# quan-dao/practical-collab-perception

Hardware: AMD Instinct MI355X
Metric: frames/sec (60k-pt cloud, 6 agents) (higher is better)
Workload: dtype f32

## Files before the change

include/pcp_hip.h:

```cpp
#ifndef PCP_HIP_H
#define PCP_HIP_H

#include <stddef.h>
#include <stdint.h>

#ifdef __cplusplus
extern "C" {
#endif

#define PCP_ABI_VERSION 1

enum {
  PCP_OK = 0,
  PCP_ERR_ARG = 1,
  PCP_ERR_WORKSPACE = 2,
  PCP_ERR_LAUNCH = 3,
  PCP_ERR_UNSUPPORTED = 4
};

int pcp_abi_version(void);
const char *pcp_status_string(int status);

enum {
  PCP_OPT_PFN_CROWD = 0,
  PCP_OPT_PFN_CROWD_BLOCKS = 1,
  PCP_OPT_PFN_WPS = 2,
  PCP_OPT_WINO4C_NW = 3,
  PCP_OPT_MP_TH16_MIN = 4,
  PCP_OPT_MP_DIAG = 5,
  PCP_OPT_VOX_AGGREGATE = 6,
  PCP_OPT_CONV_S2_FORM = 7,
  PCP_OPT_COUNT = 8
};
int pcp_set_option(int32_t option, int64_t value);
int64_t pcp_get_option(int32_t option);

typedef struct {
  float min_x, min_y, min_z;
  float voxel_x, voxel_y, voxel_z;
  int32_t nx, ny;
  int32_t batch_size;
} pcp_grid_t;

#define PCP_VOX_COUNTERS 4

size_t pcp_voxelize_workspace_bytes(const pcp_grid_t *grid, int64_t max_points);

int pcp_voxelize(const float *points, int64_t n, int32_t row_stride, const pcp_grid_t *grid,
                 void *workspace, size_t workspace_bytes,
                 int32_t *voxel_coords, int64_t *unq_inv, int32_t *unq_cnt, int32_t *counters, void *stream);
int pcp_voxelize_cells_ready(const float *points, int64_t n, int32_t row_stride, const pcp_grid_t *grid,
                             void *workspace, size_t workspace_bytes,
                             int32_t *voxel_coords, int32_t *unq_cnt, int32_t *counters, void *stream);

int pcp_voxelize_sort_pillar_rows(const pcp_grid_t *grid, void *workspace, int64_t n, void *stream);
int pcp_voxelize_row_order(const pcp_grid_t *grid, const void *workspace, int64_t n, int32_t *order, int32_t *cursor_scratch,
                           void *stream);

int pcp_pfn_scatter(const float *points, int64_t n, int32_t row_stride, int32_t num_raw, const pcp_grid_t *grid,
                    const void *workspace, const float *w0, const float *b0, const float *w1, const float *b1,
                    float *pillar_features, float *canvas, void *stream);

#define PCP_ROWS_CELLS_READY 1
#define PCP_ROWS_BUCKET_ORDER 2
size_t pcp_pillarise_rows_workspace_bytes(const pcp_grid_t *grid, int64_t max_points, int32_t num_raw);
int pcp_pillarise_rows(const float *points, int64_t n, int32_t row_stride, int32_t num_raw, const pcp_grid_t *grid,
                       void *workspace, size_t workspace_bytes, int32_t *voxel_coords, int64_t *unq_inv, int32_t *unq_cnt,
                       int32_t *counters, int32_t flags, void *stream);
int pcp_pfn_rows(const pcp_grid_t *grid, const void *workspace, int64_t n, int32_t num_raw, const float *w0, const float *b0,
                 const float *w1, const float *b1, float *pillar_features, float *canvas, void *stream);
int pcp_pillar_index_export(const pcp_grid_t *grid, const void *workspace, int64_t n, int32_t num_raw, int32_t *voxel_coords,
                            int32_t *row_rank, int32_t *slot_rank, int32_t *slot_canvas_row, int32_t *counters, void *stream);

#define PCP_PFN_ABSOLUTE_XYZ 1u
#define PCP_PFN_WITH_DISTANCE 2u
int pcp_pfn_features(const float *points, int64_t n, int32_t row_stride, int32_t num_raw, uint32_t flags, const pcp_grid_t *grid,
                     const void *vox_workspace, int32_t fw, float *fbuf, int32_t *slot_pillar, void *stream);
int pcp_pfn_cat_pillar_max(const float *y, int32_t ld_y, const float *pillar_max, int32_t ld_max, const int32_t *slot_pillar, int64_t rows,
                           int32_t c, float *out, int32_t ld_out, void *stream);

int pcp_canvas_clear(const pcp_grid_t *grid, const void *workspace, int64_t n, float *canvas, void *stream);
int pcp_fill_zero(void *ptr, size_t bytes, void *stream);

typedef struct {
  int32_t batch, in_h, in_w;
  int32_t cin, cout;
  int32_t cout_pad;
  int32_t stride;
  int32_t ld_in, ld_out;
  int32_t relu;
} pcp_conv3x3_t;

int pcp_conv3x3(const pcp_conv3x3_t *desc, const float *in, const float *w_packed, const float *bias, float *out,
                void *stream);

int pcp_sparse_conv3x3_s2(const float *pillar_features, const pcp_grid_t *grid, const void *vox_workspace, int64_t n,
                          const float *w_packed, const float *bias, int32_t cout, int32_t relu, float *out, int32_t ld_out,
                          void *stream);

int pcp_conv3x3_winograd(const pcp_conv3x3_t *desc, const float *in, const float *u_packed, const float *bias, float *out,
                         void *stream);

int pcp_conv3x3_winograd_ws_supported(const pcp_conv3x3_t *desc);
int pcp_conv3x3_winograd_ws(const pcp_conv3x3_t *desc, const float *in, const float *u_packed, const float *bias, float *out,
                            void *stream);
int pcp_conv3x3_winograd_ws_plan(const pcp_conv3x3_t *desc, int32_t *variant, double *executed_flops);

int pcp_conv3x3_winograd4f(const pcp_conv3x3_t *desc, const float *in, const float *u_packed, const float *bias, float *out,
                           void *stream);
int pcp_conv3x3_winograd4f_plan(const pcp_conv3x3_t *desc, double *executed_flops);

int pcp_conv3x3_winograd4h(const pcp_conv3x3_t *desc, const float *in, const float *u_packed, const float *bias, float *out,
                           void *stream);
int pcp_conv3x3_winograd4h_plan(const pcp_conv3x3_t *desc, double *executed_flops);

// ... 199 lines not shown
```

practical-collab-perception_amd/csrc/abi.hip:

```cpp
#include "pcp_common.h"

extern "C" int pcp_abi_version(void) { return PCP_ABI_VERSION; }

extern "C" const char *pcp_status_string(int status) {
  switch (status) {
    case PCP_OK: return "ok";
    case PCP_ERR_ARG: return "bad argument";
    case PCP_ERR_WORKSPACE: return "workspace too small";
    case PCP_ERR_LAUNCH: return "kernel launch failed";
    case PCP_ERR_UNSUPPORTED: return "unsupported shape for this build";
    default: return "unknown status";
  }
}

#include <atomic>

namespace {
std::atomic<long long> g_option[PCP_OPT_COUNT] = {{-1}, {-1}, {-1}, {-1}, {-1}, {-1}, {-1}, {-1}};
static_assert(PCP_OPT_COUNT == 8, "one initialiser per option");
constexpr int MAX_DEVICES = 64;
std::atomic<int> g_cus[MAX_DEVICES];
}

extern "C" int pcp_set_option(int32_t option, int64_t value) {
  if (option < 0 || option >= PCP_OPT_COUNT) return PCP_ERR_ARG;
  g_option[option].store(value < 0 ? -1 : (long long)value, std::memory_order_relaxed);
  return PCP_OK;
}

extern "C" int64_t pcp_get_option(int32_t option) {
  if (option < 0 || option >= PCP_OPT_COUNT) return -1;
  return g_option[option].load(std::memory_order_relaxed);
}

long long pcp_option(int option, long long builtin) {
  const long long v = g_option[option].load(std::memory_order_relaxed);
  return v < 0 ? builtin : v;
}

int pcp_current_device_cus() {
  int dev = 0;
  if (hipGetDevice(&dev) != hipSuccess || dev < 0 || dev >= MAX_DEVICES) return 256;
  int v = g_cus[dev].load(std::memory_order_relaxed);
  if (v > 0) return v;
  if (hipDeviceGetAttribute(&v, hipDeviceAttributeMultiprocessorCount, dev) != hipSuccess || v <= 0) v = 256;
  g_cus[dev].store(v, std::memory_order_relaxed);
  return v;
}
```

practical-collab-perception_amd/csrc/conv.hip:

```cpp
#include "pcp_common.h"

namespace {

constexpr int CK = 16;
constexpr int LDK = 20;
constexpr int CONV_THREADS = 256;

__device__ __forceinline__ int xcd_remap(int bid, int nwg) {
  const int q = nwg >> 3, r = nwg & 7, x = bid & 7;
  return (x < r ? x * (q + 1) : r * (q + 1) + (x - r) * q) + (bid >> 3);
}

__device__ __forceinline__ f32x16 mfma32(float a, float b, f32x16 c) {
  return __builtin_amdgcn_mfma_f32_32x32x2f32(a, b, c, 0, 0, 0);
}

struct Conv3Params {
  const float *in;
  const float *w;
  const float *bias;
  float *out;
  int batch, in_h, in_w, out_h, out_w;
  int cin, cout, cout_pad;
  int ld_in, ld_out;
// ... 269 lines not shown
  f32x4 af[2][MI];
  patch_load(0);
#pragma unroll
  for (int t = 0; t < W2_RING; t++) wr[t] = w_load(0, t);
  patch_store(0);
  patch_load(1);
  __syncthreads();
  for (int slice = 0; slice < n_slices; slice++) {
    const float *As = lds + (slice & 1) * BUF;
    patch_store((slice + 1) & 1);
    patch_load(slice + 2);
#pragma unroll
    for (int i = 0; i < MI; i++) af[0][i] = *reinterpret_cast<const f32x4 *>(As + a_off[i][0]);
    fence();
#pragma unroll
    for (int t = 0; t < 18; t++) {
      if (t + 1 < 18) {
#pragma unroll
        for (int i = 0; i < MI; i++)
          af[(t + 1) & 1][i] = *reinterpret_cast<const f32x4 *>(As + (a_off[i][(t + 1) >> 1] ^ (((t + 1) & 1) * 8)));
      }
      if (t > 0) wr[(t - 1) % W2_RING] = w_load(slice + (t - 1 + W2_RING >= 18 ? 1 : 0), (t - 1 + W2_RING) % 18);
      fence();
      const f32x4 bf = wr[t % W2_RING];
      const f32x4 a0 = af[t & 1][0], a1 = af[t & 1][1];
      acc[0] = mfma32(bf.x, a0.x, acc[0]);
      acc[1] = mfma32(bf.x, a1.x, acc[1]);
      acc[0] = mfma32(bf.y, a0.y, acc[0]);
      acc[1] = mfma32(bf.y, a1.y, acc[1]);
      acc[0] = mfma32(bf.z, a0.z, acc[0]);
      acc[1] = mfma32(bf.z, a1.z, acc[1]);
      acc[0] = mfma32(bf.w, a0.w, acc[0]);
      acc[1] = mfma32(bf.w, a1.w, acc[1]);
      fence();
    }
    wr[17 % W2_RING] = w_load(slice + 1, (17 + W2_RING) % 18);
    __syncthreads();
  }

  const int nb = n0 + wn * 32;
#pragma unroll
  for (int i = 0; i < MI; i++) {
    const int m = wm * 64 + i * 32 + r;
    const int oy = oy0 + m / TW, ox = ox0 + m % TW;
    if (oy >= p.out_h || ox >= p.out_w) continue;
    float *orow = p.out + ((long long)(b * p.out_h + oy) * p.out_w + ox) * p.ld_out;
#pragma unroll
    for (int q = 0; q < 4; q++) {
      const int co = nb + 8 * q + 4 * h;
      if (co >= p.cout) continue;
      const f32x4 bias = *reinterpret_cast<const f32x4 *>(p.bias + co);
      f32x4 v = f32x4{acc[i][4 * q], acc[i][4 * q + 1], acc[i][4 * q + 2], acc[i][4 * q + 3]} + bias;
      if (p.relu) {
        v.x = fmaxf(v.x, 0.f); v.y = fmaxf(v.y, 0.f); v.z = fmaxf(v.z, 0.f); v.w = fmaxf(v.w, 0.f);
      }
      if (co + 3 < p.cout && p.vec_out) {
        *reinterpret_cast<f32x4 *>(orow + co) = v;
      } else {
        orow[co] = v.x;
        if (co + 1 < p.cout) orow[co + 1] = v.y;
        if (co + 2 < p.cout) orow[co + 2] = v.z;
        if (co + 3 < p.cout) orow[co + 3] = v.w;
      }
    }
  }
}

struct PwParams {
  const float *in;
  const float *in2;
  const float *residual;
  int ld_in2, k_split, ld_res;
  const float *w;
  const float *bias;
  float *out;
  long long rows;
  int in_h, in_w;
  int cin, cout, cout_pad, n_total;
  int k_total;
  int ld_in, ld_out;
  int relu;
  int n_tiles;
  int vec_out;
};

template <int MODE, int BM, int BN, int WAVES_M, int WAVES_N>
__global__ __launch_bounds__(CONV_THREADS, 2) void k_pointwise(PwParams p) {
  constexpr int WTM = BM / WAVES_M, WTN = BN / WAVES_N;
  constexpr int MI = WTM / 32, NI = WTN / 32;
  constexpr int A_F4 = BM * (CK / 4), B_F4 = BN * (CK / 4);
  constexpr int A_PER = (A_F4 + CONV_THREADS - 1) / CONV_THREADS;
  constexpr int B_PER = (B_F4 + CONV_THREADS - 1) / CONV_THREADS;
  __shared__ __attribute__((aligned(16))) float lds[(BM + BN) * LDK];
  float *As = lds;
  float *Bs = lds + BM * LDK;

  const int tid = threadIdx.x, lane = tid & 63, wave = tid >> 6;
  const int r = lane & 31, h = lane >> 5;
  const int wm = wave / WAVES_N, wn = wave % WAVES_N;
  const int lid = xcd_remap(blockIdx.x, gridDim.x);
  const int nt = lid % p.n_tiles;
  const long long m0 = (long long)(lid / p.n_tiles) * BM;
  const int n0 = nt * BN;

  const float *a_row[A_PER];
  const float *a_row2[A_PER];
  int a_dst[A_PER];
#pragma unroll
  for (int i = 0; i < A_PER; i++) {
    int idx = tid + i * CONV_THREADS;
    a_row[i] = nullptr;
    a_row2[i] = nullptr;
    a_dst[i] = -1;
    if (idx < A_F4) {
      int row = idx >> 2, q = idx & 3;
      long long m = m0 + row;
      a_dst[i] = row * LDK + q * 4;
      if (m < p.rows) {
        if (MODE == PCP_PW_PLAIN && p.in2) a_row2[i] = p.in2 + m * p.ld_in2 + q * 4;
        if (MODE == PCP_PW_SPACE2DEPTH) {
          int ow = p.in_w >> 1, oh = p.in_h >> 1;
          int ox = (int)(m % ow);
          long long t = m / ow;
          int oy = (int)(t % oh), bb = (int)(t / oh);
          a_row[i] = p.in + ((long long)(bb * p.in_h + 2 * oy) * p.in_w + 2 * ox) * p.ld_in + q * 4;
        } else {
          a_row[i] = p.in + m * p.ld_in + q * 4;
        }
      }
    }
  }
  int b_goff[B_PER], b_dst[B_PER];
#pragma unroll
  for (int i = 0; i < B_PER; i++) {
    int idx = tid + i * CONV_THREADS;
    b_dst[i] = -1;
    b_goff[i] = 0;
    if (idx < B_F4) {
      int n = idx >> 2, q = idx & 3;
      b_goff[i] = (n0 + n) * CK + q * 4;
      b_dst[i] = n * LDK + q * 4;
    }
  }
  const int slices_per_tap = p.cin / CK;
  f32x4 a_reg[A_PER], b_reg[B_PER];
  auto load_slice = [&](int slice) {
    int tap = 0, c0 = slice * CK;
    long long tap_off = 0;
    if (MODE == PCP_PW_SPACE2DEPTH) {
      tap = slice / slices_per_tap;
      c0 = (slice % slices_per_tap) * CK;
      tap_off = ((long long)(tap >> 1) * p.in_w + (tap & 1)) * p.ld_in;
    }
    const bool second = (MODE == PCP_PW_PLAIN) && p.in2 && c0 >= p.k_split;
#pragma unroll
    for (int i = 0; i < A_PER; i++) {
      a_reg[i] = f32x4{0.f, 0.f, 0.f, 0.f};
      if (second) {
        if (a_row2[i]) a_reg[i] = *reinterpret_cast<const f32x4 *>(a_row2[i] + (c0 - p.k_split));
      } else if (a_row[i]) {
        a_reg[i] = *reinterpret_cast<const f32x4 *>(a_row[i] + tap_off + c0);
      }
    }
    const float *bs = p.w + (long long)slice * p.n_total * CK;
#pragma unroll
    for (int i = 0; i < B_PER; i++)
      if (b_dst[i] >= 0) b_reg[i] = *reinterpret_cast<const f32x4 *>(bs + b_goff[i]);
  };
  int a_off[MI], b_off[NI];
#pragma unroll
  for (int i = 0; i < MI; i++) a_off[i] = (wm * WTM + i * 32 + r) * LDK + 4 * h;
#pragma unroll
  for (int j = 0; j < NI; j++) b_off[j] = (wn * WTN + j * 32 + r) * LDK + 4 * h;
  f32x16 acc[MI][NI];
#pragma unroll
  for (int i = 0; i < MI; i++)
#pragma unroll
    for (int j = 0; j < NI; j++)
#pragma unroll
      for (int e = 0; e < 16; e++) acc[i][j][e] = 0.f;

  const int n_slices = p.k_total / CK;
  load_slice(0);
  for (int slice = 0; slice < n_slices; slice++) {
#pragma unroll
    for (int i = 0; i < A_PER; i++)
      if (a_dst[i] >= 0) *reinterpret_cast<f32x4 *>(As + a_dst[i]) = a_reg[i];
#pragma unroll
    for (int i = 0; i < B_PER; i++)
      if (b_dst[i] >= 0) *reinterpret_cast<f32x4 *>(Bs + b_dst[i]) = b_reg[i];
    __syncthreads();
    if (slice + 1 < n_slices) load_slice(slice + 1);
#pragma unroll
    for (int g = 0; g < CK / 8; g++) {
      f32x4 af[MI], bf[NI];
#pragma unroll
      for (int i = 0; i < MI; i++) af[i] = *reinterpret_cast<const f32x4 *>(As + a_off[i] + g * 8);
#pragma unroll
      for (int j = 0; j < NI; j++) bf[j] = *reinterpret_cast<const f32x4 *>(Bs + b_off[j] + g * 8);
#pragma unroll
      for (int i = 0; i < MI; i++)
#pragma unroll
        for (int j = 0; j < NI; j++) {
          acc[i][j] = mfma32(bf[j].x, af[i].x, acc[i][j]);
          acc[i][j] = mfma32(bf[j].y, af[i].y, acc[i][j]);
          acc[i][j] = mfma32(bf[j].z, af[i].z, acc[i][j]);
          acc[i][j] = mfma32(bf[j].w, af[i].w, acc[i][j]);
        }
    }
    __syncthreads();
  }

#pragma unroll
  for (int j = 0; j < NI; j++) {
    const int nb = n0 + wn * WTN + j * 32;
    int tap = 0, cb = nb;
    if (MODE == PCP_PW_DEPTH2SPACE) {
      tap = nb / p.cout_pad;
      cb = nb % p.cout_pad;
    }
#pragma unroll
    for (int i = 0; i < MI; i++) {
      const long long m = m0 + wm * WTM + i * 32 + r;
      if (m >= p.rows || nb >= p.n_total) continue;
      long long opix = m;
      if (MODE == PCP_PW_DEPTH2SPACE) {
        int ix = (int)(m % p.in_w);
        long long t = m / p.in_w;
        int iy = (int)(t % p.in_h), bb = (int)(t / p.in_h);
        opix = ((long long)bb * (2 * p.in_h) + 2 * iy + (tap >> 1)) * (2 * p.in_w) + 2 * ix + (tap & 1);
      }
      float *orow = p.out + opix * p.ld_out;
#pragma unroll
      for (int q = 0; q < 4; q++) {
        const int co = cb + 8 * q + 4 * h;
        if (co >= p.cout) continue;
        const f32x4 bias = *reinterpret_cast<const f32x4 *>(p.bias + co);
        f32x4 v = f32x4{acc[i][j][4 * q], acc[i][j][4 * q + 1], acc[i][j][4 * q + 2], acc[i][j][4 * q + 3]} + bias;
        if (p.relu && p.relu != PCP_RELU_PRE_RESIDUAL) {
          v.x = fmaxf(v.x, 0.f); v.y = fmaxf(v.y, 0.f); v.z = fmaxf(v.z, 0.f); v.w = fmaxf(v.w, 0.f);
        }
        if (MODE == PCP_PW_PLAIN && p.residual) {
          const float *rr = p.residual + m * p.ld_res + co;
          v.x += rr[0];
          if (co + 1 < p.cout) v.y += rr[1];
          if (co + 2 < p.cout) v.z += rr[2];
          if (co + 3 < p.cout) v.w += rr[3];
        }
        if (MODE == PCP_PW_PLAIN && p.relu == PCP_RELU_PRE_RESIDUAL) {
          v.x = fmaxf(v.x, 0.f); v.y = fmaxf(v.y, 0.f); v.z = fmaxf(v.z, 0.f); v.w = fmaxf(v.w, 0.f);
        }
        if (co + 3 < p.cout && p.vec_out) {
          *reinterpret_cast<f32x4 *>(orow + co) = v;
        } else {
          orow[co] = v.x;
          if (co + 1 < p.cout) orow[co + 1] = v.y;
          if (co + 2 < p.cout) orow[co + 2] = v.z;
          if (co + 3 < p.cout) orow[co + 3] = v.w;
        }
      }
    }
  }
}

template <int S, int TH, int TW, int BN, int WM, int WN>
int launch_conv3(const pcp_conv3x3_t *d, const float *in, const float *w, const float *bias, float *out, hipStream_t st) {
  Conv3Params p;
  p.in = in; p.w = w; p.bias = bias; p.out = out;
  p.batch = d->batch; p.in_h = d->in_h; p.in_w = d->in_w;
  p.out_h = (d->in_h + 2 - 3) / S + 1;
  p.out_w = (d->in_w + 2 - 3) / S + 1;
  p.cin = d->cin; p.cout = d->cout; p.cout_pad = d->cout_pad;
  p.ld_in = d->ld_in; p.ld_out = d->ld_out; p.relu = d->relu;
  p.tiles_x = (p.out_w + TW - 1) / TW;
  p.tiles_y = (p.out_h + TH - 1) / TH;
  p.n_tiles = d->cout_pad / BN;
  p.vec_out = (d->ld_out % 4 == 0 && (((uintptr_t)out) & 15) == 0) ? 1 : 0;
  p.in_bytes = 0;
  long long blocks = (long long)d->batch * p.tiles_x * p.tiles_y * p.n_tiles;
  if (blocks <= 0 || blocks > 0x7fffffffLL) return PCP_ERR_ARG;
  hipLaunchKernelGGL((k_conv3x3<S, TH, TW, BN, WM, WN>), dim3((unsigned)blocks), dim3(CONV_THREADS), 0, st, p);
  PCP_CHECK_LAUNCH();
  return PCP_OK;
}

long long conv3_in_bytes(const pcp_conv3x3_t *d) {
  return (((long long)d->batch * d->in_h * d->in_w - 1) * d->ld_in + d->cin) * 4;
}

template <int TH, int TW, int BN, int WM, int WN>
int launch_conv3_s2w(const pcp_conv3x3_t *d, const float *in, const float *w, const float *bias, float *out, hipStream_t st) {
  Conv3Params p;
  p.in = in; p.w = w; p.bias = bias; p.out = out;
  p.batch = d->batch; p.in_h = d->in_h; p.in_w = d->in_w;
  p.out_h = (d->in_h - 1) / 2 + 1;
  p.out_w = (d->in_w - 1) / 2 + 1;
  p.cin = d->cin; p.cout = d->cout; p.cout_pad = d->cout_pad;
  p.ld_in = d->ld_in; p.ld_out = d->ld_out; p.relu = d->relu;
  p.tiles_x = (p.out_w + TW - 1) / TW;
  p.tiles_y = (p.out_h + TH - 1) / TH;
  p.n_tiles = d->cout_pad / BN;
  p.vec_out = (d->ld_out % 4 == 0 && (((uintptr_t)out) & 15) == 0) ? 1 : 0;
  p.in_bytes = (unsigned)conv3_in_bytes(d);
  long long blocks = (long long)d->batch * p.tiles_x * p.tiles_y * p.n_tiles;
  if (blocks <= 0 || blocks > 0x7fffffffLL) return PCP_ERR_ARG;
  hipLaunchKernelGGL((k_conv3x3_s2w<TH, TW, BN, WM, WN>), dim3((unsigned)blocks), dim3(CONV_THREADS), 0, st, p);
  PCP_CHECK_LAUNCH();
  return PCP_OK;
}

template <int MODE, int BM, int BN, int WM, int WN>
int launch_pw(const PwParams &p0, hipStream_t st) {
  PwParams p = p0;
  p.n_tiles = (p.n_total + BN - 1) / BN;
  long long blocks = ((p.rows + BM - 1) / BM) * p.n_tiles;
  if (blocks <= 0 || blocks > 0x7fffffffLL) return PCP_ERR_ARG;
  hipLaunchKernelGGL((k_pointwise<MODE, BM, BN, WM, WN>), dim3((unsigned)blocks), dim3(CONV_THREADS), 0, st, p);
  PCP_CHECK_LAUNCH();
  return PCP_OK;
}

}

extern "C" int pcp_conv3x3(const pcp_conv3x3_t *d, const float *in, const float *w_packed, const float *bias, float *out,
                           void *stream_) {
  if (!d || !in || !w_packed || !bias || !out) return PCP_ERR_ARG;
  if (d->cin <= 0 || d->cin % CK != 0 || d->cout <= 0 || d->cout_pad < d->cout || d->cout_pad % 32 != 0) return PCP_ERR_ARG;
  if (d->ld_in % 4 != 0 || (((uintptr_t)in) & 15) || (((uintptr_t)w_packed) & 15) || (((uintptr_t)bias) & 15)) return PCP_ERR_ARG;
  if (d->batch <= 0 || d->in_h <= 0 || d->in_w <= 0) return PCP_ERR_ARG;
  hipStream_t st = (hipStream_t)stream_;
  if (d->stride == 1) {
    if (d->cout_pad % 64 == 0) return launch_conv3<1, 8, 16, 64, 2, 2>(d, in, w_packed, bias, out, st);
    return launch_conv3<1, 8, 16, 32, 4, 1>(d, in, w_packed, bias, out, st);
  } else if (d->stride == 2) {
    if (d->cout_pad % 64 == 0) {
      const long long form = pcp_option(PCP_OPT_CONV_S2_FORM, 0);
      if (form != 0 && form != 1 && form != 2) return PCP_ERR_ARG;
      const bool fits = conv3_in_bytes(d) <= 0x7fffffffLL;
      if (form == 2 && !fits) return PCP_ERR_UNSUPPORTED;
      if (form != 1 && fits) {
        if (d->cout_pad % 128 == 0) return launch_conv3_s2w<8, 8, 128, 1, 4>(d, in, w_packed, bias, out, st);
        return launch_conv3_s2w<8, 16, 64, 2, 2>(d, in, w_packed, bias, out, st);
      }
      return launch_conv3<2, 8, 8, 64, 2, 2>(d, in, w_packed, bias, out, st);
    }
    return launch_conv3<2, 8, 16, 32, 4, 1>(d, in, w_packed, bias, out, st);
  }
  return PCP_ERR_UNSUPPORTED;
}

extern "C" int pcp_pointwise(const pcp_pointwise_t *d, const float *in, const float *w_packed, const float *bias, float *out,
                             void *stream_) {
  if (!d || !in || !w_packed || !bias || !out) return PCP_ERR_ARG;
  if (d->cin <= 0 || d->cin % CK != 0 || d->cout <= 0 || d->cout_pad < d->cout || d->cout_pad % 32 != 0) return PCP_ERR_ARG;
  if (d->ld_in % 4 != 0 || (((uintptr_t)in) & 15) || (((uintptr_t)w_packed) & 15) || (((uintptr_t)bias) & 15)) return PCP_ERR_ARG;
  hipStream_t st = (hipStream_t)stream_;
  PwParams p;
  p.in = in; p.w = w_packed; p.bias = bias; p.out = out;
  p.in2 = nullptr; p.residual = nullptr; p.ld_in2 = 0; p.k_split = 0; p.ld_res = 0;
  if (d->mode == PCP_PW_PLAIN) {
    p.in2 = d->in2; p.ld_in2 = d->ld_in2; p.k_split = d->k_split;
    p.residual = d->residual; p.ld_res = d->ld_res;
    if (p.in2 && (p.k_split <= 0 || p.k_split % CK != 0 || p.k_split >= d->cin || (p.ld_in2 & 3) || (((uintptr_t)p.in2) & 15)))
      return PCP_ERR_ARG;
  }
  if (d->relu == PCP_RELU_PRE_RESIDUAL && (d->mode != PCP_PW_PLAIN || !d->residual)) return PCP_ERR_ARG;
  p.in_h = d->in_h; p.in_w = d->in_w;
  p.cin = d->cin; p.cout = d->cout; p.cout_pad = d->cout_pad;
  p.ld_in = d->ld_in; p.ld_out = d->ld_out; p.relu = d->relu;
  p.n_tiles = 0;
  p.vec_out = (d->ld_out % 4 == 0 && (((uintptr_t)out) & 15) == 0) ? 1 : 0;
  switch (d->mode) {
    case PCP_PW_PLAIN:
      if (d->rows <= 0) return d->rows == 0 ? PCP_OK : PCP_ERR_ARG;
      p.rows = d->rows; p.k_total = d->cin; p.n_total = d->cout_pad;
      if (d->cout_pad % 64 == 0) return launch_pw<PCP_PW_PLAIN, 128, 64, 2, 2>(p, st);
      return launch_pw<PCP_PW_PLAIN, 128, 32, 4, 1>(p, st);
    case PCP_PW_SPACE2DEPTH:
      if (d->batch <= 0 || d->in_h <= 0 || d->in_w <= 0 || (d->in_h & 1) || (d->in_w & 1)) return PCP_ERR_ARG;
      p.rows = (long long)d->batch * (d->in_h / 2) * (d->in_w / 2);
      p.k_total = 4 * d->cin; p.n_total = d->cout_pad;
      if (d->cout_pad % 64 == 0) return launch_pw<PCP_PW_SPACE2DEPTH, 128, 64, 2, 2>(p, st);
      return launch_pw<PCP_PW_SPACE2DEPTH, 128, 32, 4, 1>(p, st);
    case PCP_PW_DEPTH2SPACE:
      if (d->batch <= 0 || d->in_h <= 0 || d->in_w <= 0) return PCP_ERR_ARG;
      p.rows = (long long)d->batch * d->in_h * d->in_w;
      p.k_total = d->cin; p.n_total = 4 * d->cout_pad;
      if (d->cout_pad % 64 == 0) return launch_pw<PCP_PW_DEPTH2SPACE, 128, 64, 2, 2>(p, st);
      return launch_pw<PCP_PW_DEPTH2SPACE, 128, 32, 4, 1>(p, st);
    default:
      return PCP_ERR_UNSUPPORTED;
  }
}
```

practical-collab-perception_amd/pcp_amd/lib.py:

```python
import ctypes
import os

_HERE = os.path.dirname(os.path.abspath(__file__))
LIB_PATH = os.environ.get('PCP_HIP_LIB') or os.path.abspath(os.path.join(_HERE, '..', 'lib', 'libpcp_hip.so'))

c_f = ctypes.c_float
c_i32 = ctypes.c_int32
c_i64 = ctypes.c_int64
c_sz = ctypes.c_size_t
vp = ctypes.c_void_p


class Grid(ctypes.Structure):
    _fields_ = [('min_x', c_f), ('min_y', c_f), ('min_z', c_f), ('voxel_x', c_f), ('voxel_y', c_f), ('voxel_z', c_f),
                ('nx', c_i32), ('ny', c_i32), ('batch_size', c_i32)]


class PackJob(ctypes.Structure):
    _fields_ = [('w', ctypes.c_void_p), ('cout', ctypes.c_int32), ('cin', ctypes.c_int32), ('transpose', ctypes.c_int32),
                ('direct_cout_pad', ctypes.c_int32), ('direct', ctypes.c_void_p), ('winograd', ctypes.c_void_p),
                ('winograd_cout_pad', ctypes.c_int32), ('f4_cout_pad', ctypes.c_int32), ('u4f', ctypes.c_void_p), ('u4h', ctypes.c_void_p),
                ('block_start', ctypes.c_int32), ('reserved', ctypes.c_int32)]


# ... 238 lines not shown
    'pcp_centerhead_loss': (c_i32, [ctypes.POINTER(HeadLoss), vp, vp, vp, vp, vp, c_f, vp, vp, vp, vp]),
    'pcp_centerhead_targets_ext': (c_i32, [ctypes.POINTER(Target), ctypes.POINTER(TargetHead), c_i32, vp, c_i32, c_i32, c_i32, vp]),
    'pcp_centerhead_loss_ext_workspace_bytes': (c_sz, [c_i32]),
    'pcp_centerhead_loss_ext': (c_i32, [ctypes.POINTER(HeadLossExt), ctypes.POINTER(HeadLossHead), c_i32, c_f, vp, c_sz, vp, vp, vp]),
    'pcp_anchor_assign_workspace_bytes': (c_sz, [ctypes.POINTER(AnchorAssign), c_i32]),
    'pcp_anchor_assign_targets': (c_i32, [ctypes.POINTER(AnchorAssign), vp, vp, c_i32, vp, c_sz, vp, vp, vp, vp]),
    'pcp_anchor_loss_workspace_bytes': (c_sz, [c_i32]),
    'pcp_anchor_loss': (c_i32, [ctypes.POINTER(AnchorLoss), vp, vp, vp, vp, c_f, vp, c_sz, vp, vp, vp]),
    'pcp_hunter_meta_workspace_bytes': (c_sz, [ctypes.POINTER(HunterMeta), c_i64]),
    'pcp_hunter_meta': (c_i32, [ctypes.POINTER(HunterMeta), vp, c_i64, c_i32, vp, c_sz, vp, vp, vp, vp, vp, vp, vp, vp, vp]),
    'pcp_segment_max': (c_i32, [vp, c_i32, vp, c_i64, vp, c_i64, c_i32, vp, c_i32, vp, vp]),
    'pcp_segment_max_backward': (c_i32, [vp, c_i32, vp, c_i64, c_i32, vp, vp, c_i32, vp]),
    'pcp_rows_scatter_add': (c_i32, [vp, c_i32, vp, c_i64, c_i32, vp, c_i32, vp]),
    'pcp_hunter_local_centroids': (c_i32, [vp, c_i32, vp, vp, c_i32, c_i32, vp, c_sz, vp, vp, c_i32, vp]),
    'pcp_hunter_object_cat': (c_i32, [vp, vp, vp, vp, vp, c_i32, c_i32, vp, c_i32, vp]),
    'pcp_hunter_object_cat_backward': (c_i32, [vp, c_i32, vp, vp, c_i32, c_i32, c_i32, vp, vp, vp]),
    'pcp_hunter_loss_workspace_bytes': (c_sz, [c_i64, c_i32, c_i32, c_i32]),
    'pcp_hunter_losses': (c_i32, [ctypes.POINTER(HunterLoss), vp, c_sz, vp]),
    'pcp_softmax_fuse2_backward': (c_i32, [vp, c_i32, vp, c_i32, vp, c_i32, c_i64, c_i32, vp, c_i32, vp, c_i32, vp]),
    'pcp_bev_scatter_mean_backward': (c_i32, [vp, c_i32, c_i32, c_i32, c_i64, vp, c_i32, c_i32, vp, vp, c_i32, vp, c_i32, vp]),
    'pcp_bev_sample_bilinear_backward': (c_i32, [vp, c_i32, vp, vp, c_i64, c_i32, vp, c_i32, c_i32, c_i32, c_i32, c_i32, c_f, c_f, c_f, c_f, vp,
                                                 c_i32, vp, c_i32, vp]),
    'pcp_filter_gt_boxes': (c_i32, [vp, c_i32, c_i32, ctypes.POINTER(c_f), vp, vp]),
    'pcp_distill_loss': (c_i32, [vp, c_i32, vp, c_i32, c_i64, c_i32, c_f, c_f, vp, vp, vp, c_i32, c_i32, vp]),
    'pcp_masked_smooth_l1_rows': (c_i32, [vp, c_i32, vp, c_i32, c_i64, c_i32, c_f, vp, vp, vp]),
    'pcp_pfn_train_features': (c_i32, [vp, c_i64, c_i32, c_i32, ctypes.POINTER(Grid), vp, vp, vp, vp]),
    'pcp_pfn_train_features_w': (c_i32, [vp, c_i64, c_i32, c_i32, c_i32, ctypes.POINTER(Grid), vp, vp, vp, vp]),
    'pcp_pfn_train_mid': (c_i32, [ctypes.POINTER(Grid), vp, c_i64, vp, vp, vp, vp, vp, vp]),
    'pcp_pfn_train_out': (c_i32, [ctypes.POINTER(Grid), vp, c_i64, vp, vp, vp, vp, vp, vp, vp]),
    'pcp_pfn_train_route_out_grad': (c_i32, [ctypes.POINTER(Grid), vp, c_i64, c_i64, vp, vp, vp, vp, vp]),
    'pcp_pfn_train_route_mid_grad': (c_i32, [ctypes.POINTER(Grid), vp, c_i64, vp, vp, vp, vp]),
    'pcp_disco_weight_logits': (c_i32, [ctypes.POINTER(vp), c_i32, c_i32, vp, vp, c_i64, vp, c_i32, vp]),
    'pcp_disco_fuse_backward_workspace_bytes': (c_sz, []),
    'pcp_disco_fuse_backward': (c_i32, [ctypes.POINTER(vp), c_i32, c_i32, c_i32, vp, c_i32, vp, c_i32, ctypes.POINTER(vp), c_i32, vp,
                                        c_i64, vp, c_i32, ctypes.POINTER(vp), vp, vp, vp, c_i32, vp]),
    'pcp_grad_sqnorm': (c_i32, [vp, c_i64, vp, c_i32, vp]),
    'pcp_pack_conv3x3': (c_i32, [vp, c_i32, c_i32, c_i32, vp, c_i32, vp, c_i32, vp, c_i32, vp]),
    'pcp_pack_conv3x3_winograd4': (c_i32, [vp, c_i32, c_i32, c_i32, vp, vp, c_i32, vp]),
    'pcp_pack_conv3x3_group_blocks': (c_i32, [vp]),
    'pcp_pack_conv3x3_group': (c_i32, [vp, c_i32, c_i32, vp]),
    'pcp_adam_step': (c_i32, [vp, vp, vp, vp, c_i64, c_f, c_f, c_f, c_f, c_f, c_i64, c_f, vp, c_f, vp]),
    'pcp_avgpool_nhwc_backward': (c_i32, [vp, c_i32, c_i32, c_i32, c_i32, c_i32, c_i32, vp, c_i32, c_i32, vp]),
    'pcp_sc_gate_backward': (c_i32, [vp, c_i32, vp, c_i32, vp, c_i32, vp, c_i32, c_i32, c_i32, vp, c_i32, vp, c_i32, vp, c_i32, c_i32, vp, c_i32,
                                     c_i32, c_i32, c_i32, c_i32, vp]),
    'pcp_add_relu': (c_i32, [vp, c_i32, vp, c_i32, vp, c_i32, c_i64, c_i32, vp]),
    'pcp_add_relu_backward': (c_i32, [vp, c_i32, vp, c_i32, vp, c_i32, vp, c_i32, c_i64, c_i32, vp]),
})

SYMBOLS.update({
    'pcp_mp_bn_train_stats': (c_i32, [vp, c_i32, c_i64, c_i32, c_i32, vp, vp, c_f, c_f, vp, vp, vp, vp, vp, vp, vp, vp]),
    'pcp_mp_scale_shift_act': (c_i32, [vp, c_i32, c_i64, c_i32, c_i32, vp, vp, c_i32, vp, c_i32, c_i32, vp]),
    'pcp_mp_bn_act_backward': (c_i32, [vp, c_i32, c_i32, vp, c_i32, c_i32, c_i64, c_i32, vp, vp, vp, vp, c_i32, vp, vp, vp, c_i32, vp, c_i32,
                                       c_i32, vp]),
    'pcp_mp_bn_train_sums': (c_i32, [vp, c_i32, c_i64, c_i32, c_i32, vp, vp, vp]),
    'pcp_mp_bn_bwd_sums': (c_i32, [vp, c_i32, c_i32, vp, c_i32, c_i32, c_i64, c_i32, vp, vp, vp, vp, c_i32, vp, vp, vp]),
    'pcp_mp_bn_bwd_apply_from_sums': (c_i32, [vp, c_i32, c_i32, vp, c_i32, c_i32, c_i64, c_i32, vp, vp, vp, vp, c_i32, vp, vp, c_i64, vp, vp, vp,
                                              c_i32, vp, c_i32, c_i32, vp]),
    'pcp_mp_colsum': (c_i32, [vp, c_i32, c_i64, c_i32, c_i32, vp, vp, c_i32, vp]),
    'pcp_mp_accumulate': (c_i32, [vp, c_i32, c_i32, vp, c_i32, c_i32, c_i64, c_i32, c_f, vp]),
    'pcp_mp_dilate2x': (c_i32, [vp, c_i32, c_i32, c_i32, c_i32, c_i32, c_i32, vp, c_i32, vp]),
    'pcp_mp_pfn_train_mid': (c_i32, [ctypes.POINTER(Grid), vp, c_i64, vp, vp, vp, vp, c_i32, vp, vp]),
    'pcp_mp_pfn_train_out': (c_i32, [ctypes.POINTER(Grid), vp, c_i64, vp, c_i32, vp, vp, vp, vp, vp, c_i32, vp]),
    'pcp_mp_pfn_train_route_out_grad': (c_i32, [ctypes.POINTER(Grid), vp, c_i64, c_i64, vp, c_i32, vp, vp, vp, c_i32, vp]),
    'pcp_mp_pfn_train_route_mid_grad': (c_i32, [ctypes.POINTER(Grid), vp, c_i64, vp, c_i32, vp, vp, vp]),
    'pcp_mp_sparse_conv3x3_s2': (c_i32, [vp, ctypes.POINTER(Grid), vp, c_i64, vp, vp, c_i32, c_i32, vp, c_i32, c_i32, vp]),
    'pcp_mp_conv3x3_packed_bytes': (c_sz, [c_i32, c_i32]),
    'pcp_mp_pack_conv3x3': (c_i32, [vp, c_i32, c_i32, c_i32, vp, vp, c_i32, vp]),
    'pcp_mp_pack_conv3x3_group_blocks': (c_i32, [vp]),
    'pcp_mp_pack_conv3x3_group': (c_i32, [vp, c_i32, c_i32, vp]),
    'pcp_mp_conv3x3': (c_i32, [ctypes.POINTER(MpConv3x3), vp, vp, vp, vp, vp]),
    'pcp_mp_conv3x3_plan': (c_i32, [ctypes.POINTER(MpConv3x3), ctypes.POINTER(c_i32), ctypes.POINTER(ctypes.c_double)]),
    'pcp_mp_conv3x3_wgrad_workspace_bytes': (c_sz, [ctypes.POINTER(MpWgrad3x3)]),
    'pcp_mp_conv3x3_wgrad': (c_i32, [ctypes.POINTER(MpWgrad3x3), vp, vp, vp, vp, c_sz, vp]),
    'pcp_mp_pointwise': (c_i32, [ctypes.POINTER(MpPointwise), vp, vp, vp, vp, vp]),
    'pcp_mp_warp_nearest': (c_i32, [vp, c_i32, vp, c_i32, c_i32, c_i32, c_i32, c_i32, c_i32, ctypes.POINTER(c_f), c_i32, vp]),
    'pcp_mp_softmax_fuse': (c_i32, [ctypes.POINTER(vp), c_i32, c_i32, vp, c_i32, c_i64, c_i32, c_i32, c_i32, vp, vp]),
    'pcp_mp_disco_fuse_backward': (c_i32, [ctypes.POINTER(vp), c_i32, c_i32, c_i32, c_i32, vp, c_i32, vp, c_i32, ctypes.POINTER(vp), c_i32, vp, c_i64,
                                           vp, c_i32, ctypes.POINTER(vp), vp, vp, vp, c_i32, vp]),
    'pcp_mp_pointwise_wgrad_workspace_bytes': (c_sz, [c_i64, c_i32, c_i32]),
    'pcp_mp_pointwise_wgrad': (c_i32, [ctypes.POINTER(MpRowMap), ctypes.POINTER(MpRowMap), c_i64, vp, c_sz, vp, c_i32, c_i32, vp]),
})

OPTIONS = {'pfn_crowd': 0, 'pfn_crowd_blocks': 1, 'pfn_wps': 2, 'wino4c_nw': 3, 'mp_th16_min': 4, 'mp_diag': 5, 'vox_aggregate': 6,
           'conv_s2_form': 7}
_OPTION_ENV = {'PCP_PFN_CROWD': 'pfn_crowd', 'PCP_PFN_CROWD_BLOCKS': 'pfn_crowd_blocks', 'PCP_PFN_WPS': 'pfn_wps', 'PCP_WINO4C_NW': 'wino4c_nw',
               'PCP_MP_TH16_MIN': 'mp_th16_min', 'PCP_MP_DIAG': 'mp_diag', 'PCP_VOX_AGGREGATE': 'vox_aggregate', 'PCP_CONV_S2_FORM': 'conv_s2_form'}

_LIB = None


class PcpError(RuntimeError):
    pass


def load():
    global _LIB
    if _LIB is not None:
        return _LIB
    if not os.path.isfile(LIB_PATH):
        raise PcpError('libpcp_hip.so not found at %s -- build it with `make -C practical-collab-perception_amd/csrc` '
                       '(or python -c "import __graft_entry__ as g; g.build()"); there is no CPU fallback.' % LIB_PATH)
    import torch
    lib = ctypes.CDLL(LIB_PATH)
    for name, (res, args) in SYMBOLS.items():
        fn = getattr(lib, name)
        fn.restype = res
        fn.argtypes = args
    if lib.pcp_abi_version() != 1:
        raise PcpError('libpcp_hip.so ABI version mismatch')
    for env, name in _OPTION_ENV.items():
        v = os.environ.get(env, '')
        if v.strip():
            if lib.pcp_set_option(OPTIONS[name], int(v)) != 0:
                raise PcpError('%s=%s: pcp_set_option refused it' % (env, v))
    _LIB = lib
    return lib


def set_option(name, value):
    lib = load()
    prev = int(lib.pcp_get_option(OPTIONS[name]))
    check(lib.pcp_set_option(OPTIONS[name], -1 if value is None else int(value)), 'pcp_set_option')
    return None if prev < 0 else prev


def check(status, what):
    if status != 0:
        raise PcpError('%s failed: %s' % (what, load().pcp_status_string(status).decode()))
```

Baseline: 403.9.

## Add register-pipelined pointwise GEMM kernel with buffer loads and swizzled LDS

Adds a new pointwise-conv kernel variant. It double-buffers only the activation tile in swizzled LDS and streams weights straight from global memory into registers two slices ahead, using buffer loads with hardware bounds checks. A heuristic picks this kernel by tile count per CU round (smaller tiles for small grids, the wide form for large space-to-depth), and an option can force either path. The aim is to cut LDS traffic and barrier stalls in the pointwise GEMMs. The cost is more register pressure and an extra selection rule that may misroute some shapes.

```diff
diff --git a/include/pcp_hip.h b/include/pcp_hip.h
--- a/include/pcp_hip.h
+++ b/include/pcp_hip.h
@@ -30,7 +30,8 @@
   PCP_OPT_MP_DIAG = 5,
   PCP_OPT_VOX_AGGREGATE = 6,
   PCP_OPT_CONV_S2_FORM = 7,
-  PCP_OPT_COUNT = 8
+  PCP_OPT_PW_FORM = 8,
+  PCP_OPT_COUNT = 9
 };
 int pcp_set_option(int32_t option, int64_t value);
 int64_t pcp_get_option(int32_t option);
diff --git a/practical-collab-perception_amd/csrc/abi.hip b/practical-collab-perception_amd/csrc/abi.hip
--- a/practical-collab-perception_amd/csrc/abi.hip
+++ b/practical-collab-perception_amd/csrc/abi.hip
@@ -16,8 +16,8 @@
 #include <atomic>
 
 namespace {
-std::atomic<long long> g_option[PCP_OPT_COUNT] = {{-1}, {-1}, {-1}, {-1}, {-1}, {-1}, {-1}, {-1}};
-static_assert(PCP_OPT_COUNT == 8, "one initialiser per option");
+std::atomic<long long> g_option[PCP_OPT_COUNT] = {{-1}, {-1}, {-1}, {-1}, {-1}, {-1}, {-1}, {-1}, {-1}};
+static_assert(PCP_OPT_COUNT == 9, "one initialiser per option");
 constexpr int MAX_DEVICES = 64;
 std::atomic<int> g_cus[MAX_DEVICES];
 }
diff --git a/practical-collab-perception_amd/csrc/conv.hip b/practical-collab-perception_amd/csrc/conv.hip
--- a/practical-collab-perception_amd/csrc/conv.hip
+++ b/practical-collab-perception_amd/csrc/conv.hip
@@ -375,7 +375,10 @@
   int relu;
   int n_tiles;
   int vec_out;
+  unsigned in_bytes, in2_bytes, w_bytes;
 };
+
+typedef f32x4 f32x4_a4 __attribute__((aligned(4)));
 
 template <int MODE, int BM, int BN, int WAVES_M, int WAVES_N>
 __global__ __launch_bounds__(CONV_THREADS, 2) void k_pointwise(PwParams p) {
@@ -450,9 +453,9 @@
     for (int i = 0; i < A_PER; i++) {
       a_reg[i] = f32x4{0.f, 0.f, 0.f, 0.f};
       if (second) {
-        if (a_row2[i]) a_reg[i] = *reinterpret_cast<const f32x4 *>(a_row2[i] + (c0 - p.k_split));
+        if (a_row2[i]) a_reg[i] = *reinterpret_cast<const f32x4_a4 *>(a_row2[i] + (c0 - p.k_split));
       } else if (a_row[i]) {
-        a_reg[i] = *reinterpret_cast<const f32x4 *>(a_row[i] + tap_off + c0);
+        a_reg[i] = *reinterpret_cast<const f32x4_a4 *>(a_row[i] + tap_off + c0);
       }
     }
     const float *bs = p.w + (long long)slice * p.n_total * CK;
@@ -515,6 +518,209 @@
 #pragma unroll
     for (int i = 0; i < MI; i++) {
       const long long m = m0 + wm * WTM + i * 32 + r;
+      if (m >= p.rows || nb >= p.n_total) continue;
+      long long opix = m;
+      if (MODE == PCP_PW_DEPTH2SPACE) {
+        int ix = (int)(m % p.in_w);
+        long long t = m / p.in_w;
+        int iy = (int)(t % p.in_h), bb = (int)(t / p.in_h);
+        opix = ((long long)bb * (2 * p.in_h) + 2 * iy + (tap >> 1)) * (2 * p.in_w) + 2 * ix + (tap & 1);
+      }
+      float *orow = p.out + opix * p.ld_out;
+#pragma unroll
+      for (int q = 0; q < 4; q++) {
+        const int co = cb + 8 * q + 4 * h;
+        if (co >= p.cout) continue;
+        const f32x4 bias = *reinterpret_cast<const f32x4 *>(p.bias + co);
+        f32x4 v = f32x4{acc[i][j][4 * q], acc[i][j][4 * q + 1], acc[i][j][4 * q + 2], acc[i][j][4 * q + 3]} + bias;
+        if (p.relu && p.relu != PCP_RELU_PRE_RESIDUAL) {
+          v.x = fmaxf(v.x, 0.f); v.y = fmaxf(v.y, 0.f); v.z = fmaxf(v.z, 0.f); v.w = fmaxf(v.w, 0.f);
+        }
+        if (MODE == PCP_PW_PLAIN && p.residual) {
+          const float *rr = p.residual + m * p.ld_res + co;
+          v.x += rr[0];
+          if (co + 1 < p.cout) v.y += rr[1];
+          if (co + 2 < p.cout) v.z += rr[2];
+          if (co + 3 < p.cout) v.w += rr[3];
+        }
+        if (MODE == PCP_PW_PLAIN && p.relu == PCP_RELU_PRE_RESIDUAL) {
+          v.x = fmaxf(v.x, 0.f); v.y = fmaxf(v.y, 0.f); v.z = fmaxf(v.z, 0.f); v.w = fmaxf(v.w, 0.f);
+        }
+        if (co + 3 < p.cout && p.vec_out) {
+          *reinterpret_cast<f32x4 *>(orow + co) = v;
+        } else {
+          orow[co] = v.x;
+          if (co + 1 < p.cout) orow[co + 1] = v.y;
+          if (co + 2 < p.cout) orow[co + 2] = v.z;
+          if (co + 3 < p.cout) orow[co + 3] = v.w;
+        }
+      }
+    }
+  }
+}
+
+template <int V>
+struct PwBuf { static constexpr int value = V; };
+
+template <int MODE, int WAVES_M, int WAVES_N, int NI>
+__global__ __launch_bounds__(CONV_THREADS, 2) void k_pointwise_w(PwParams p) {
+  constexpr int MI = 2;
+  constexpr int BM = WAVES_M * MI * 32, BN = WAVES_N * NI * 32;
+  constexpr int BUF = BM * CK;
+  constexpr int A_PER = BM * (CK / 4) / CONV_THREADS;
+  constexpr int T = 2 * NI;
+  static_assert(WAVES_M * WAVES_N * 64 == CONV_THREADS && A_PER * CONV_THREADS == BM * (CK / 4), "every thread stages A_PER 16-byte items");
+
+  __shared__ __attribute__((aligned(16))) float lds[2 * BUF];
+
+  const int tid = threadIdx.x;
+  const int lane = tid & 63;
+  const int wave = __builtin_amdgcn_readfirstlane(tid >> 6);
+  const int r = lane & 31, h = lane >> 5;
+  const int wm = wave / WAVES_N, wn = wave % WAVES_N;
+  const int lid = xcd_remap(blockIdx.x, gridDim.x);
+  const int nt = lid % p.n_tiles;
+  const long long m0 = (long long)(lid / p.n_tiles) * BM;
+  const int n0 = nt * BN;
+
+  const __amdgpu_buffer_rsrc_t in_rsrc = __builtin_amdgcn_make_buffer_rsrc(const_cast<float *>(p.in), 0, p.in_bytes, 0x00020000);
+  const __amdgpu_buffer_rsrc_t in2_rsrc = __builtin_amdgcn_make_buffer_rsrc(const_cast<float *>(p.in2), 0, p.in2_bytes, 0x00020000);
+  const bool dual = MODE == PCP_PW_PLAIN && p.in2 != nullptr;
+  unsigned a_goff[A_PER], a_goff2[A_PER];
+  int a_dst[A_PER];
+#pragma unroll
+  for (int i = 0; i < A_PER; i++) {
+    const int idx = tid + i * CONV_THREADS;
+    const int row = idx >> 2, q = idx & 3;
+    const long long m = m0 + row;
+    a_dst[i] = row * CK + ((q ^ ((row >> 2) & 3)) << 2);
+    a_goff[i] = 0x80000000u;
+    a_goff2[i] = 0x80000000u;
+    if (m < p.rows) {
+      long long pix = m;
+      if (MODE == PCP_PW_SPACE2DEPTH) {
+        const int ow = p.in_w >> 1, oh = p.in_h >> 1;
+        const int ox = (int)(m % ow);
+        const long long t = m / ow;
+        const int oy = (int)(t % oh), bb = (int)(t / oh);
+        pix = (long long)(bb * p.in_h + 2 * oy) * p.in_w + 2 * ox;
+      }
+      a_goff[i] = (unsigned)((pix * p.ld_in + q * 4) * 4);
+      if (dual) a_goff2[i] = (unsigned)((m * p.ld_in2 + q * 4) * 4);
+    }
+  }
+  const int n_slices = p.k_total / CK;
+  const int last = n_slices - 1;
+  int ld_slice = 0, ld_c0 = 0, ld_tap = 0, ld_tap_off = 0;
+  f32x4 a_reg[A_PER];
+  auto row_load = [&]() {
+    const bool second = dual && ld_c0 >= p.k_split;
+    const __amdgpu_buffer_rsrc_t rsrc = second ? in2_rsrc : in_rsrc;
+    const int soff = second ? (ld_c0 - p.k_split) * 4 : ld_c0 * 4 + ld_tap_off;
+#pragma unroll
+    for (int i = 0; i < A_PER; i++)
+      a_reg[i] = __builtin_bit_cast(f32x4, __builtin_amdgcn_raw_buffer_load_b128(rsrc, (int)(second ? a_goff2[i] : a_goff[i]), soff, 0));
+    if (ld_slice < last) {
+      ld_slice++;
+      ld_c0 += CK;
+      if (MODE == PCP_PW_SPACE2DEPTH && ld_c0 == p.cin) {
+        ld_c0 = 0;
+        ld_tap++;
+        ld_tap_off = ((ld_tap >> 1) * p.in_w + (ld_tap & 1)) * p.ld_in * 4;
+      }
+    }
+  };
+  auto row_store = [&](int buf) {
+    float *dst = lds + buf * BUF;
+#pragma unroll
+    for (int i = 0; i < A_PER; i++) *reinterpret_cast<f32x4 *>(dst + a_dst[i]) = a_reg[i];
+  };
+
+  const __amdgpu_buffer_rsrc_t w_rsrc = __builtin_amdgcn_make_buffer_rsrc(const_cast<float *>(p.w), 0, p.w_bytes, 0x00020000);
+  const int w_voff = ((n0 + wn * NI * 32 + r) * CK + 4 * h) * 4;
+  const int w_slice = p.n_total * CK * 4;
+  auto w_load = [&](int slice, int f) {
+    return __builtin_bit_cast(f32x4, __builtin_amdgcn_raw_buffer_load_b128(w_rsrc, w_voff + (f % NI) * 32 * CK * 4 + (f / NI) * 32,
+                                                                           min(slice, last) * w_slice, 0));
+  };
+
+  int a_off[MI];
+#pragma unroll
+  for (int i = 0; i < MI; i++) {
+    const int ml = (wm * MI + i) * 32 + r;
+    a_off[i] = ml * CK + ((h ^ ((ml >> 2) & 3)) << 2);
+  }
+
+  f32x16 acc[MI][NI];
+#pragma unroll
+  for (int i = 0; i < MI; i++)
+#pragma unroll
+    for (int j = 0; j < NI; j++)
+#pragma unroll
+      for (int e = 0; e < 16; e++) acc[i][j][e] = 0.f;
+
+  const auto fence = [] { __builtin_amdgcn_sched_barrier(0); };
+  f32x4 wr[2][T];
+  f32x4 af[2][MI];
+  auto slice_step = [&](auto pb, int slice) {
+    constexpr int P = decltype(pb)::value;
+    const float *As = lds + P * BUF;
+    row_store(P ^ 1);
+    row_load();
+#pragma unroll
+    for (int i = 0; i < MI; i++) af[0][i] = *reinterpret_cast<const f32x4 *>(As + a_off[i]);
+    fence();
+#pragma unroll
+    for (int f = 0; f < T; f++) {
+      if (f == 0) {
+#pragma unroll
+        for (int i = 0; i < MI; i++) af[1][i] = *reinterpret_cast<const f32x4 *>(As + (a_off[i] ^ 8));
+      }
+      if (f > 0) wr[P][f - 1] = w_load(slice + 2, f - 1);
+      fence();
+      const int g = f / NI, j = f % NI;
+      const f32x4 bf = wr[P][f];
+      const f32x4 a0 = af[g][0], a1 = af[g][1];
+      acc[0][j] = mfma32(bf.x, a0.x, acc[0][j]);
+      acc[1][j] = mfma32(bf.x, a1.x, acc[1][j]);
+      acc[0][j] = mfma32(bf.y, a0.y, acc[0][j]);
+      acc[1][j] = mfma32(bf.y, a1.y, acc[1][j]);
+      acc[0][j] = mfma32(bf.z, a0.z, acc[0][j]);
+      acc[1][j] = mfma32(bf.z, a1.z, acc[1][j]);
+      acc[0][j] = mfma32(bf.w, a0.w, acc[0][j]);
+      acc[1][j] = mfma32(bf.w, a1.w, acc[1][j]);
+      fence();
+    }
+    wr[P][T - 1] = w_load(slice + 2, T - 1);
+    __syncthreads();
+  };
+
+  row_load();
+#pragma unroll
+  for (int f = 0; f < T; f++) wr[0][f] = w_load(0, f);
+#pragma unroll
+  for (int f = 0; f < T; f++) wr[1][f] = w_load(1, f);
+  row_store(0);
+  row_load();
+  __syncthreads();
+  int slice = 0;
+  for (; slice + 1 < n_slices; slice += 2) {
+    slice_step(PwBuf<0>{}, slice);
+    slice_step(PwBuf<1>{}, slice + 1);
+  }
+  if (slice < n_slices) slice_step(PwBuf<0>{}, slice);
+
+#pragma unroll
+  for (int j = 0; j < NI; j++) {
+    const int nb = n0 + (wn * NI + j) * 32;
+    int tap = 0, cb = nb;
+    if (MODE == PCP_PW_DEPTH2SPACE) {
+      tap = nb / p.cout_pad;
+      cb = nb % p.cout_pad;
+    }
+#pragma unroll
+    for (int i = 0; i < MI; i++) {
+      const long long m = m0 + (wm * MI + i) * 32 + r;
       if (m >= p.rows || nb >= p.n_total) continue;
       long long opix = m;
       if (MODE == PCP_PW_DEPTH2SPACE) {
@@ -613,6 +819,49 @@
   return PCP_OK;
 }
 
+template <int MODE, int WM, int WN, int NI>
+int launch_pw_w(const PwParams &p0, hipStream_t st) {
+  constexpr int BM = WM * 64, BN = WN * NI * 32;
+  PwParams p = p0;
+  p.n_tiles = p.n_total / BN;
+  long long blocks = ((p.rows + BM - 1) / BM) * p.n_tiles;
+  if (blocks <= 0 || blocks > 0x7fffffffLL) return PCP_ERR_ARG;
+  hipLaunchKernelGGL((k_pointwise_w<MODE, WM, WN, NI>), dim3((unsigned)blocks), dim3(CONV_THREADS), 0, st, p);
+  PCP_CHECK_LAUNCH();
+  return PCP_OK;
+}
+
+template <int MODE>
+int launch_pw_mode(const PwParams &p, int wide, hipStream_t st) {
+  if (wide) {
+    if (p.n_total % 128 == 0 && wide == 1) return launch_pw_w<MODE, 2, 2, 2>(p, st);
+    if (p.n_total % 64 == 0) return launch_pw_w<MODE, 2, 2, 1>(p, st);
+    return launch_pw_w<MODE, 4, 1, 1>(p, st);
+  }
+  if (p.cout_pad % 64 == 0) return launch_pw<MODE, 128, 64, 2, 2>(p, st);
+  return launch_pw<MODE, 128, 32, 4, 1>(p, st);
+}
+
+int pw_rule(int mode, const PwParams &p) {
+  if (p.n_total % 64 != 0) return 0;
+  const long long round = 4LL * pcp_current_device_cus();
+  const long long m_tiles = (p.rows + 127) / 128;
+  if (mode == PCP_PW_SPACE2DEPTH) return (p.n_total % 128 == 0 && m_tiles * (p.n_total / 128) > round) ? 1 : 0;
+  return m_tiles * (p.n_total / 64) <= round ? 2 : 0;
+}
+
+bool pw_wide_fits(PwParams *p, long long pixels) {
+  if (p->ld_in % 4 != 0 || (((uintptr_t)p->in) & 15)) return false;
+  const long long lim = 0x7fffffffLL;
+  if (pixels > lim || p->rows > lim) return false;
+  const long long in_b = ((pixels - 1) * p->ld_in + (p->in2 ? p->k_split : p->cin)) * 4;
+  const long long in2_b = p->in2 ? ((p->rows - 1) * p->ld_in2 + (p->cin - p->k_split)) * 4 : 0;
+  const long long w_b = (long long)(p->k_total / CK) * p->n_total * CK * 4;
+  if (in_b > lim || in2_b > lim || w_b > lim) return false;
+  p->in_bytes = (unsigned)in_b; p->in2_bytes = (unsigned)in2_b; p->w_bytes = (unsigned)w_b;
+  return true;
+}
+
 }
 
 extern "C" int pcp_conv3x3(const pcp_conv3x3_t *d, const float *in, const float *w_packed, const float *bias, float *out,
@@ -646,7 +895,9 @@
                              void *stream_) {
   if (!d || !in || !w_packed || !bias || !out) return PCP_ERR_ARG;
   if (d->cin <= 0 || d->cin % CK != 0 || d->cout <= 0 || d->cout_pad < d->cout || d->cout_pad % 32 != 0) return PCP_ERR_ARG;
-  if (d->ld_in % 4 != 0 || (((uintptr_t)in) & 15) || (((uintptr_t)w_packed) & 15) || (((uintptr_t)bias) & 15)) return PCP_ERR_ARG;
+  if ((((uintptr_t)in) & 3) || (((uintptr_t)w_packed) & 15) || (((uintptr_t)bias) & 15)) return PCP_ERR_ARG;
+  const long long form = pcp_option(PCP_OPT_PW_FORM, 0);
+  if (form != 0 && form != 1 && form != 2) return PCP_ERR_ARG;
   hipStream_t st = (hipStream_t)stream_;
   PwParams p;
   p.in = in; p.w = w_packed; p.bias = bias; p.out = out;
@@ -663,24 +914,22 @@
   p.ld_in = d->ld_in; p.ld_out = d->ld_out; p.relu = d->relu;
   p.n_tiles = 0;
   p.vec_out = (d->ld_out % 4 == 0 && (((uintptr_t)out) & 15) == 0) ? 1 : 0;
+  p.in_bytes = p.in2_bytes = p.w_bytes = 0;
   switch (d->mode) {
     case PCP_PW_PLAIN:
       if (d->rows <= 0) return d->rows == 0 ? PCP_OK : PCP_ERR_ARG;
       p.rows = d->rows; p.k_total = d->cin; p.n_total = d->cout_pad;
-      if (d->cout_pad % 64 == 0) return launch_pw<PCP_PW_PLAIN, 128, 64, 2, 2>(p, st);
-      return launch_pw<PCP_PW_PLAIN, 128, 32, 4, 1>(p, st);
+      return launch_pw_mode<PCP_PW_PLAIN>(p, form == 1 || !pw_wide_fits(&p, p.rows) ? 0 : form == 2 ? 1 : pw_rule(PCP_PW_PLAIN, p), st);
     case PCP_PW_SPACE2DEPTH:
       if (d->batch <= 0 || d->in_h <= 0 || d->in_w <= 0 || (d->in_h & 1) || (d->in_w & 1)) return PCP_ERR_ARG;
       p.rows = (long long)d->batch * (d->in_h / 2) * (d->in_w / 2);
       p.k_total = 4 * d->cin; p.n_total = d->cout_pad;
-      if (d->cout_pad % 64 == 0) return launch_pw<PCP_PW_SPACE2DEPTH, 128, 64, 2, 2>(p, st);
-      return launch_pw<PCP_PW_SPACE2DEPTH, 128, 32, 4, 1>(p, st);
+      return launch_pw_mode<PCP_PW_SPACE2DEPTH>(p, form == 1 || !pw_wide_fits(&p, (long long)d->batch * d->in_h * d->in_w) ? 0 : form == 2 ? 1 : pw_rule(PCP_PW_SPACE2DEPTH, p), st);
     case PCP_PW_DEPTH2SPACE:
       if (d->batch <= 0 || d->in_h <= 0 || d->in_w <= 0) return PCP_ERR_ARG;
       p.rows = (long long)d->batch * d->in_h * d->in_w;
       p.k_total = d->cin; p.n_total = 4 * d->cout_pad;
-      if (d->cout_pad % 64 == 0) return launch_pw<PCP_PW_DEPTH2SPACE, 128, 64, 2, 2>(p, st);
-      return launch_pw<PCP_PW_DEPTH2SPACE, 128, 32, 4, 1>(p, st);
+      return launch_pw_mode<PCP_PW_DEPTH2SPACE>(p, form == 1 || !pw_wide_fits(&p, p.rows) ? 0 : form == 2 ? 1 : pw_rule(PCP_PW_DEPTH2SPACE, p), st);
     default:
       return PCP_ERR_UNSUPPORTED;
   }
diff --git a/practical-collab-perception_amd/pcp_amd/lib.py b/practical-collab-perception_amd/pcp_amd/lib.py
--- a/practical-collab-perception_amd/pcp_amd/lib.py
+++ b/practical-collab-perception_amd/pcp_amd/lib.py
@@ -344,9 +344,10 @@
 })
 
 OPTIONS = {'pfn_crowd': 0, 'pfn_crowd_blocks': 1, 'pfn_wps': 2, 'wino4c_nw': 3, 'mp_th16_min': 4, 'mp_diag': 5, 'vox_aggregate': 6,
-           'conv_s2_form': 7}
+           'conv_s2_form': 7, 'pw_form': 8}
 _OPTION_ENV = {'PCP_PFN_CROWD': 'pfn_crowd', 'PCP_PFN_CROWD_BLOCKS': 'pfn_crowd_blocks', 'PCP_PFN_WPS': 'pfn_wps', 'PCP_WINO4C_NW': 'wino4c_nw',
-               'PCP_MP_TH16_MIN': 'mp_th16_min', 'PCP_MP_DIAG': 'mp_diag', 'PCP_VOX_AGGREGATE': 'vox_aggregate', 'PCP_CONV_S2_FORM': 'conv_s2_form'}
+               'PCP_MP_TH16_MIN': 'mp_th16_min', 'PCP_MP_DIAG': 'mp_diag', 'PCP_VOX_AGGREGATE': 'vox_aggregate', 'PCP_CONV_S2_FORM': 'conv_s2_form',
+               'PCP_PW_FORM': 'pw_form'}
 
 _LIB = None
 
```

After: 403.4 (median of 2 runs). Within noise of the previous version (-0.1%).
